# Pixie8888/R3DFSSeg

Measured on NVIDIA B200. Metric: MPTI episodes/s (2-way 5-shot, 2048 pts), higher is better.
Workload: dtype f32

## Files before the change

r3dfsseg_b200/csrc/api.cu:

```cuda
#include <stdlib.h>

#include "common.cuh"
#include "lp.cuh"
#include "proto.cuh"
#include "episode.cuh"

__global__ void gather_clouds_kernel(const float* __restrict__ x, int clouds_in, int C, int N,
                                     int64_t s_g, int64_t s_cloud, int64_t s_c, int64_t s_n,
                                     int cpe_out, int cloud_off, float* __restrict__ out,
                                     int64_t total) {
  const int64_t e = (int64_t)blockIdx.x * blockDim.x + threadIdx.x;
  if (e >= total) return;
  const int c = (int)(e % C);
  int64_t r = e / C;
  const int n = (int)(r % N);
  r /= N;
  const int cl = (int)(r % clouds_in);
  const int64_t grp = r / clouds_in;
  const int64_t ocloud = grp * cpe_out + cloud_off + cl;
  out[(ocloud * N + n) * C + c] = x[grp * s_g + cl * s_cloud + c * s_c + n * s_n];
}

__global__ void copy_cols_kernel(const float* __restrict__ src, int lds, int64_t M, int ncols,
                                 float* __restrict__ dst, int ldd, RowMap map) {
// ... 31 lines not shown
__global__ void proto_rows_kernel(const float* __restrict__ proto, int64_t p_e,
                                  const int32_t* __restrict__ proto_count, int64_t c_e, int S,
                                  int slot, int ppad, int64_t f_rows, float* __restrict__ F,
                                  int32_t* __restrict__ proto_cnt) {
  constexpr int D4 = R3DFS_FEAT_DIM / 4;
  const int e = blockIdx.y;
  const int i = blockIdx.x * blockDim.x + threadIdx.x;
  if (i < S) proto_cnt[e * S + i] = min(max(proto_count[e * c_e + i], 0), slot);
  if (i >= ppad * D4) return;
  const int r = i / D4, s = r / slot;
  int cnt = 0;
  if (s < S) cnt = min(max(proto_count[e * c_e + s], 0), slot);
  float4 v = make_float4(0.f, 0.f, 0.f, 0.f);
  if (r - s * slot < cnt) v = reinterpret_cast<const float4*>(proto + e * p_e)[i];
  reinterpret_cast<float4*>(F + e * f_rows * R3DFS_FEAT_DIM)[i] = v;
}

__global__ void i32_to_i64_kernel(const int32_t* __restrict__ a, int64_t* __restrict__ b,
                                  int64_t n) {
  const int64_t e = (int64_t)blockIdx.x * blockDim.x + threadIdx.x;
  if (e < n) b[e] = a[e];
}

thread_local long long r3dfs_launches = 0;

bool simt_gemm_forced() {
  static const bool v = [] {
    const char* e = R3DFS_GETENV("R3DFS_SIMT_GEMM");
    return e && e[0] == '1';
  }();
  return v;
}

int launch_knn_auto(const float* x, int ld, int C, const float* xx, int64_t B, int N, int k,
                    int32_t* idx32, int64_t* idx64, int impl, cudaStream_t st, void* split_ws,
                    size_t split_bytes) {
  if (impl == 2)
    return launch_knn_tc(x, ld, C, xx, B, N, k, idx32, idx64, st, split_ws, split_bytes);
  if (impl == 0 && !simt_gemm_forced() && C <= 64)
    return launch_knn_tc(x, ld, C, xx, B, N, k, idx32, idx64, st, split_ws, split_bytes);
  return launch_knn(x, ld, C, xx, B, N, k, idx32, idx64, st);
}

int launch_edge_mlp_auto(const float* PQ, const int32_t* idx, const float* w2, const float* s2,
                         const float* t2, int64_t B, int N, int k, float* Y, int ldy, RowMap map,
                         cudaStream_t st) {
  if (simt_gemm_forced())
    return launch_edge_mlp(PQ, idx, w2, s2, t2, B, N, k, Y, ldy, map, nullptr, st);
  return launch_edge_mlp_tc(PQ, idx, w2, s2, t2, B, N, k, Y, ldy, map, st);
}

int launch_attention_auto(const float* qkv, int ld, int64_t B, int N, float* Y, int ldy,
                          RowMap map, cudaStream_t st, float* kmax_ws, void* split_ws,
                          size_t split_bytes) {
  if (simt_gemm_forced()) return launch_attention(qkv, ld, B, N, Y, ldy, map, st);
  return launch_attention_tc(qkv, ld, B, N, Y, ldy, map, st, kmax_ws, split_ws, split_bytes);
}

int launch_linear_auto(const float* X, int ldx, const float* W, const float* s, const float* t,
                       int act, int64_t M, int K, int Nout, float* Y, int ldy, RowMap map,
                       cudaStream_t st) {
  if (simt_gemm_forced())
    return launch_linear(X, ldx, W, s, t, act, M, K, Nout, Y, ldy, map, st);
  const int rc = launch_linear_tma(X, ldx, W, s, t, act, M, K, Nout, Y, ldy, map, st);
  if (rc != R3DFS_E_UNSUPPORTED) return rc;
  return launch_linear_tc(X, ldx, W, s, t, act, M, K, Nout, Y, ldy, map, st);
}

static inline unsigned nblk(int64_t n, int t = 256) { return (unsigned)((n + t - 1) / t); }

void carve_encoder(WsBump& ws, int64_t M, int k, EncoderWs& e) {
  e.xx = ws.take<float>(M);
  e.idx = ws.take<int32_t>(M * k);
// ... 2 lines not shown
  e.tpq = ws.take<float>(128);
  e.PQ = ws.take<float>(M * 128);
  e.ecat = ws.take<float>(M * 192);
  e.h512 = ws.take<float>(M * 512);
  e.l2 = ws.take<float>(M * 256);
  e.h128 = ws.take<float>(M * 128);
  e.qkv = ws.take<float>(M * 192);
}

int check_weights(const r3dfs_weights_t* w) {
  if (!w) return R3DFS_E_BADARG;
  if (w->in_dim < 1 || w->in_dim > 64 || w->dgcnn_k < 1 || w->dgcnn_k > 32)
    return R3DFS_E_UNSUPPORTED;
  for (int i = 0; i < 3; ++i)
    if (!w->ec_w1[i] || !w->ec_s1[i] || !w->ec_t1[i] || !w->ec_w2[i] || !w->ec_s2[i] ||
        !w->ec_t2[i])
      return R3DFS_E_BADARG;
  for (int i = 0; i < 2; ++i)
    if (!w->mlp_w[i] || !w->mlp_s[i] || !w->mlp_t[i] || !w->bl_w[i] || !w->bl_s[i] || !w->bl_t[i])
      return R3DFS_E_BADARG;
  if (!w->att_wqkv) return R3DFS_E_BADARG;
  return 0;
}

int encoder_forward(const r3dfs_weights_t* w, const float* xp, int64_t B, int N,
                           const EncoderWs& e, float* F, RowMap map, float* level2,
                           cudaStream_t st, const StageRec* sr) {
  const int64_t M = B * N;
  const int k = w->dgcnn_k;
  for (int i = 0; i < 3; ++i) {
    const float* in = i == 0 ? xp : e.ecat + 64 * (i - 1);
    const int ld = i == 0 ? w->in_dim : 192;
    const int C = i == 0 ? w->in_dim : 64;
    R3DFS_TRY(launch_row_norms(in, M, ld, C, e.xx, st));
    R3DFS_TRY(launch_knn_auto(in, ld, C, e.xx, B, N, k, e.idx, nullptr, 0, st, e.h512,
                              sizeof(float) * (size_t)M * 512));
    if (sr) sr->mark(R3DFS_ST_KNN0 + 3 * i, st);
    R3DFS_TRY(launch_fold_edge_w1(w->ec_w1[i], w->ec_s1[i], w->ec_t1[i], C, e.wpq, e.spq, e.tpq, st));
    R3DFS_TRY(launch_linear_auto(in, ld, e.wpq, e.spq, e.tpq, ACT_NONE, M, C, 128, e.PQ, 128,
                            identity_map(), st));
    if (sr) sr->mark(R3DFS_ST_PQ0 + 3 * i, st);
    R3DFS_TRY(launch_edge_mlp_auto(e.PQ, e.idx, w->ec_w2[i], w->ec_s2[i], w->ec_t2[i], B, N, k,
                                   e.ecat + 64 * i, 192, identity_map(), st));
    if (sr) sr->mark(R3DFS_ST_EDGE0 + 3 * i, st);
  }
  copy_cols_kernel<<<nblk(M * 16), 256, 0, st>>>(e.ecat, 192, M, 64, F, 192, map);
  R3DFS_CHECK_LAUNCH();
  R3DFS_TRY(launch_linear_auto(e.ecat, 192, w->mlp_w[0], w->mlp_s[0], w->mlp_t[0], ACT_LRELU, M, 192,
                          512, e.h512, 512, identity_map(), st));
  R3DFS_TRY(launch_linear_auto(e.h512, 512, w->mlp_w[1], w->mlp_s[1], w->mlp_t[1], ACT_LRELU, M, 512,
                          256, e.l2, 256, identity_map(), st));
  if (sr) sr->mark(R3DFS_ST_MLP, st);
  if (level2) {
    cudaError_t ce = cudaMemcpyAsync(level2, e.l2, sizeof(float) * M * 256,
                                     cudaMemcpyDeviceToDevice, st);
    if (ce != cudaSuccess) return (int)ce;
  }
  R3DFS_TRY(launch_linear_auto(e.l2, 256, w->bl_w[0], w->bl_s[0], w->bl_t[0], ACT_RELU, M, 256, 128,
                          e.h128, 128, identity_map(), st));
  R3DFS_TRY(launch_linear_auto(e.h128, 128, w->bl_w[1], w->bl_s[1], w->bl_t[1], ACT_NONE, M, 128, 64,
                          F + 128, 192, map, st));
  if (sr) sr->mark(R3DFS_ST_BASE, st);
  R3DFS_TRY(launch_linear_auto(e.l2, 256, w->att_wqkv, nullptr, nullptr, ACT_NONE, M, 256, 192, e.qkv,
                          192, identity_map(), st));
  if (sr) sr->mark(R3DFS_ST_QKV, st);
  R3DFS_TRY(launch_attention_auto(e.qkv, 192, B, N, F + 64, 192, map, st, e.xx, e.h512,
                                  sizeof(float) * (size_t)M * 512));
// ... 14 lines not shown
    case R3DFS_E_UNSUPPORTED: return "shape not supported by the sm_100a kernels";
    case R3DFS_E_WORKSPACE: return "workspace too small";
    case R3DFS_E_ALIGN: return "pointer not 16-byte aligned";
    default: break;
  }
  if (code > 0) return cudaGetErrorString((cudaError_t)code);
  return "unknown error";
}

size_t r3dfs_knn_workspace(int64_t B, int64_t C, int64_t N, int k) {
  return align_up(sizeof(float) * B * N * C, 256) + align_up(sizeof(float) * B * N, 256) +
         align_up(knn_split_bytes((int)C, B, (int)N, k), 256) + 768;
}

int r3dfs_knn(const float* x, int64_t B, int64_t C, int64_t N, int64_t sb, int64_t sc, int64_t sn,
              int k, int64_t* idx_out, void* wsp, size_t ws_bytes, r3dfs_stream_t stream) {
  return r3dfs_knn_ex(x, B, C, N, sb, sc, sn, k, idx_out, 0, wsp, ws_bytes, stream);
}

int r3dfs_knn_ex(const float* x, int64_t B, int64_t C, int64_t N, int64_t sb, int64_t sc,
                 int64_t sn, int k, int64_t* idx_out, int impl, void* wsp, size_t ws_bytes,
                 r3dfs_stream_t stream) {
  if (!x || !idx_out || !wsp || B <= 0 || C <= 0 || N <= 0) return R3DFS_E_BADARG;
  if (k < 1 || k > 32 || k > N) return R3DFS_E_UNSUPPORTED;
  if (ws_bytes < r3dfs_knn_workspace(B, C, N, k)) return R3DFS_E_WORKSPACE;
  cudaStream_t st = (cudaStream_t)stream;
  WsBump ws(wsp, ws_bytes);
  float* xp = ws.take<float>(B * N * C);
  float* xx = ws.take<float>(B * N);
  const size_t split_bytes = knn_split_bytes((int)C, B, (int)N, k);
  unsigned char* split = split_bytes ? ws.take<unsigned char>(split_bytes) : nullptr;
  if (!ws.ok()) return R3DFS_E_WORKSPACE;
  R3DFS_TRY(launch_to_point_major(x, B, C, N, sb, sc, sn, xp, st));
  R3DFS_TRY(launch_row_norms(xp, B * N, (int)C, (int)C, xx, st));
  if (impl < 0 || impl > 2) return R3DFS_E_UNSUPPORTED;
  return launch_knn_auto(xp, (int)C, (int)C, xx, B, (int)N, k, nullptr, idx_out, impl, st, split,
                         split_bytes);
}

size_t r3dfs_edge_feature_workspace(int64_t B, int64_t C, int64_t N) {
  return edge_feature_scratch_bytes(B, C, N);
}

int r3dfs_edge_feature(const float* x, int64_t B, int64_t C, int64_t N, int64_t sb, int64_t sc,
                       int64_t sn, const int64_t* idx, int K, float* out, void* ws, size_t ws_bytes,
                       r3dfs_stream_t stream) {
  if (!x || !idx || !out || B <= 0 || C <= 0 || N <= 0 || K <= 0) return R3DFS_E_BADARG;
  if (C > 65535 || B > 65535) return R3DFS_E_UNSUPPORTED;
  if (((uintptr_t)out & 15) != 0) return R3DFS_E_ALIGN;
  return launch_edge_feature(x, B, C, N, sb, sc, sn, idx, K, out, (cudaStream_t)stream, ws, ws_bytes);
}

int r3dfs_linear_ex(const float* x, int64_t ldx, const float* w, const float* s, const float* t,
                    int act, int64_t M, int64_t K, int64_t Nout, float* y, int64_t ldy, int impl,
                    r3dfs_stream_t stream) {
  if (!x || !w || !y || M <= 0 || K <= 0 || Nout <= 0 || ldx < K || ldy < Nout)
    return R3DFS_E_BADARG;
  if (act < 0 || act > 2 || Nout > 65535 * 64 || impl < 0 || impl > 3) return R3DFS_E_UNSUPPORTED;
  cudaStream_t st = (cudaStream_t)stream;
  if (impl == 1)
    return launch_linear(x, (int)ldx, w, s, t, act, M, (int)K, (int)Nout, y, (int)ldy,
                         identity_map(), st);
  if (impl == 2)
    return launch_linear_tc(x, (int)ldx, w, s, t, act, M, (int)K, (int)Nout, y, (int)ldy,
                            identity_map(), st);
  if (impl == 3)
    return launch_linear_tma(x, (int)ldx, w, s, t, act, M, (int)K, (int)Nout, y, (int)ldy,
// ... 9 lines not shown
}

size_t r3dfs_edgeconv_workspace(int64_t B, int64_t C, int64_t N, int k) {
  const int64_t M = B * N;
  return align_up(sizeof(float) * M * C, 256) + align_up(sizeof(float) * M, 256) +
         align_up(sizeof(int32_t) * M * k, 256) + align_up(sizeof(float) * 128 * C, 256) +
         2 * 512 + align_up(sizeof(float) * M * 128, 256) +
         align_up(knn_split_bytes((int)C, B, (int)N, k), 256) + 1280;
}

int r3dfs_edgeconv(const float* x, int64_t B, int64_t C, int64_t N, int64_t sb, int64_t sc,
                   int64_t sn, int k, const float* w1, const float* s1, const float* t1,
                   const float* w2, const float* s2, const float* t2, float* y, int64_t* idx_out,
                   void* wsp, size_t ws_bytes, r3dfs_stream_t stream) {
  if (!x || !w1 || !s1 || !t1 || !w2 || !s2 || !t2 || !y || !wsp || B <= 0 || C <= 0 || N <= 0)
    return R3DFS_E_BADARG;
  if (k < 1 || k > 32 || k > N || B > 65535) return R3DFS_E_UNSUPPORTED;
  if (ws_bytes < r3dfs_edgeconv_workspace(B, C, N, k)) return R3DFS_E_WORKSPACE;
  if (((uintptr_t)y & 15) != 0) return R3DFS_E_ALIGN;
  cudaStream_t st = (cudaStream_t)stream;
  const int64_t M = B * N;
  WsBump ws(wsp, ws_bytes);
  float* xp = ws.take<float>(M * C);
  float* xx = ws.take<float>(M);
  int32_t* idx = ws.take<int32_t>(M * k);
  float* wpq = ws.take<float>(128 * C);
  float* spq = ws.take<float>(128);
  float* tpq = ws.take<float>(128);
  float* PQ = ws.take<float>(M * 128);
  const size_t split_bytes = knn_split_bytes((int)C, B, (int)N, k);
  unsigned char* split = split_bytes ? ws.take<unsigned char>(split_bytes) : nullptr;
  if (!ws.ok()) return R3DFS_E_WORKSPACE;
  R3DFS_TRY(launch_to_point_major(x, B, C, N, sb, sc, sn, xp, st));
  R3DFS_TRY(launch_row_norms(xp, M, (int)C, (int)C, xx, st));
  R3DFS_TRY(launch_knn_auto(xp, (int)C, (int)C, xx, B, (int)N, k, idx, idx_out, 0, st, split,
                            split_bytes));
  R3DFS_TRY(launch_fold_edge_w1(w1, s1, t1, (int)C, wpq, spq, tpq, st));
  R3DFS_TRY(launch_linear_auto(xp, (int)C, wpq, spq, tpq, ACT_NONE, M, (int)C, 128, PQ, 128,
                               identity_map(), st));
  return launch_edge_mlp_auto(PQ, idx, w2, s2, t2, B, (int)N, k, y, 64, identity_map(), st);
}

size_t r3dfs_attention_workspace(int64_t B, int64_t N) {
  return align_up(sizeof(float) * B * N * 192, 256) + align_up(sizeof(float) * B, 256) +
         align_up(attention_split_bytes(B, (int)N), 256) + 512;
}

int r3dfs_attention(const float* x, int64_t B, int64_t N, int64_t Cin, const float* wqkv, float* y,
                    void* wsp, size_t ws_bytes, r3dfs_stream_t stream) {
  if (!x || !wqkv || !y || !wsp || B <= 0 || N <= 0 || Cin <= 0) return R3DFS_E_BADARG;
  if (B > 65535) return R3DFS_E_UNSUPPORTED;
  if (ws_bytes < r3dfs_attention_workspace(B, N)) return R3DFS_E_WORKSPACE;
  cudaStream_t st = (cudaStream_t)stream;
  WsBump ws(wsp, ws_bytes);
  float* qkv = ws.take<float>(B * N * 192);
  float* kmax = ws.take<float>(B);
  const size_t split_bytes = attention_split_bytes(B, (int)N);
  unsigned char* split = ws.take<unsigned char>(split_bytes);
  if (!ws.ok()) return R3DFS_E_WORKSPACE;
  R3DFS_TRY(launch_linear_auto(x, (int)Cin, wqkv, nullptr, nullptr, ACT_NONE, B * N, (int)Cin, 192,
                               qkv, 192, identity_map(), st));
  return launch_attention_auto(qkv, 192, B, (int)N, y, 64, identity_map(), st, kmax, split,
                               split_bytes);
}

size_t r3dfs_features_workspace(int64_t B, int64_t N) {
  const int64_t M = B * N;
// ... 654 lines not shown
```

r3dfsseg_b200/csrc/common.cuh:

```cuda
#pragma once
#include <cuda_runtime.h>
#include <stdint.h>
#include <math.h>

#include "../../include/r3dfs.h"

#define R3DFS_FEAT_DIM 192
#define R3DFS_EC_WIDTH 64

extern thread_local long long r3dfs_launches;

#ifdef R3DFS_AB_SWITCHES
#include <stdlib.h>
#define R3DFS_GETENV(name) getenv(name)
#else
#define R3DFS_GETENV(name) ((const char*)nullptr)
#endif

#define R3DFS_CHECK_LAUNCH()                       \
  do {                                             \
    cudaError_t e__ = cudaGetLastError();          \
    if (e__ != cudaSuccess) return (int)e__;       \
    ++r3dfs_launches;                              \
  } while (0)
// ... 41 lines not shown
  int cpe;
  int n;
  int64_t ep_rows;
  int64_t row_off;
  __host__ __device__ inline int64_t operator()(int64_t m) const {
    if (cpe == 0) return m;
    int64_t b = m / n, i = m - b * n;
    return (b / cpe) * ep_rows + row_off + (b % cpe) * (int64_t)n + i;
  }
};
static inline RowMap identity_map() { return RowMap{0, 1, 0, 0}; }

enum Act { ACT_NONE = 0, ACT_RELU = 1, ACT_LRELU = 2 };

__device__ __forceinline__ float apply_act(float v, int act) {
  if (act == ACT_RELU) return fmaxf(v, 0.f);
  if (act == ACT_LRELU) return v > 0.f ? v : 0.2f * v;
  return v;
}

__device__ __forceinline__ float warp_sum(float v) {
#pragma unroll
  for (int o = 16; o > 0; o >>= 1) v += __shfl_xor_sync(0xffffffffu, v, o);
  return v;
}

int launch_to_point_major(const float* x, int64_t B, int64_t C, int64_t N, int64_t sb, int64_t sc,
                          int64_t sn, float* out, cudaStream_t st);
int launch_row_norms(const float* x, int64_t rows, int ld, int C, float* out, cudaStream_t st);
int launch_row_norms_batched(const float* x, int64_t xs, int batch, int64_t rows, int ld, int C,
                             float* out, cudaStream_t st);
int launch_knn(const float* x, int ld, int C, const float* xx, int64_t B, int N, int k,
               int32_t* idx32, int64_t* idx64, cudaStream_t st);
int launch_knn_tc(const float* x, int ld, int C, const float* xx, int64_t B, int N, int k,
                  int32_t* idx32, int64_t* idx64, cudaStream_t st, void* split_ws = nullptr,
                  size_t split_bytes = 0);
size_t knn_split_bytes(int C, int64_t B, int N, int k);
int launch_knn_auto(const float* x, int ld, int C, const float* xx, int64_t B, int N, int k,
                    int32_t* idx32, int64_t* idx64, int impl, cudaStream_t st,
                    void* split_ws = nullptr, size_t split_bytes = 0);
int launch_linear(const float* X, int ldx, const float* W, const float* s, const float* t, int act,
                  int64_t M, int K, int Nout, float* Y, int ldy, RowMap map, cudaStream_t st);
int launch_linear_tc(const float* X, int ldx, const float* W, const float* s, const float* t,
                     int act, int64_t M, int K, int Nout, float* Y, int ldy, RowMap map,
                     cudaStream_t st);
int launch_linear_tma(const float* X, int ldx, const float* W, const float* s, const float* t,
                      int act, int64_t M, int K, int Nout, float* Y, int ldy, RowMap map,
                      cudaStream_t st);
int launch_linear_auto(const float* X, int ldx, const float* W, const float* s, const float* t,
                       int act, int64_t M, int K, int Nout, float* Y, int ldy, RowMap map,
                       cudaStream_t st);
int launch_gram_dist_ts(const float* F, int64_t graph_rows, int64_t row_off, int G, int nn, int D,
                        const float* norms, float* D2, cudaStream_t st);
int launch_gram_dist_tc(const float* F, int64_t graph_rows, int64_t row_off, int G, int nn, int D,
                        const float* norms, float* D2, cudaStream_t st);
int launch_edge_mlp_tc(const float* PQ, const int32_t* idx, const float* w2, const float* s2,
                       const float* t2, int64_t B, int N, int k, float* Y, int ldy, RowMap map,
                       cudaStream_t st);
int launch_edge_mlp_auto(const float* PQ, const int32_t* idx, const float* w2, const float* s2,
                         const float* t2, int64_t B, int N, int k, float* Y, int ldy, RowMap map,
                         cudaStream_t st);
bool simt_gemm_forced();
int launch_edge_mlp(const float* PQ, const int32_t* idx, const float* w2, const float* s2,
                    const float* t2, int64_t B, int N, int k, float* Y, int ldy, RowMap map,
                    float* w2t_scratch, cudaStream_t st);
int launch_edge_feature(const float* x, int64_t B, int64_t C, int64_t N, int64_t sb, int64_t sc,
                        int64_t sn, const int64_t* idx, int K, float* out, cudaStream_t st,
                        void* ws = nullptr, size_t ws_bytes = 0);
size_t edge_feature_scratch_bytes(int64_t B, int64_t C, int64_t N);
int launch_attention(const float* qkv, int ld, int64_t B, int N, float* Y, int ldy, RowMap map,
                     cudaStream_t st);
// ... 18 lines not shown
```

r3dfsseg_b200/csrc/tc_knn.cu:

```cuda
#include <stdlib.h>

#include "common.cuh"
#include "tc.cuh"

#define KT_TQ 128
#define KT_TC 128
#define KT_THREADS 384

template <int KC4>
struct KnnTcSmem {
  static constexpr int TILE = tc::tile_bytes(128, KC4);
  static constexpr int Q_OFF = 0;
  static constexpr int B_OFF = 2 * TILE;
  static constexpr int QV_OFF = B_OFF + 4 * TILE;
  static constexpr int QI_OFF = QV_OFF + 16 * 256 * 4;
  static constexpr int XS_OFF = QI_OFF + 16 * 256;
  static constexpr int TOTAL = XS_OFF + 4 * 128 * 4 + 64;
};

template <int KC4>
__device__ __forceinline__ void knn_store_tile(unsigned char* hi_base, unsigned char* lo_base,
                                               const float* __restrict__ x, int ld, int C,
                                               int64_t row0, int64_t rows_end, int t, int nthr,
                                               bool vec_ok) {
// ... 57 lines not shown
template <int KC4, int ROWS, int NTHR>
__device__ __forceinline__ void tile_store(const TileRegs<KC4, ROWS, NTHR>& tr,
                                           unsigned char* hi_base, unsigned char* lo_base, int t) {
  constexpr int LBO = tc::tile_lbo(ROWS);
#pragma unroll
  for (int i = 0; i < TileRegs<KC4, ROWS, NTHR>::NCH; ++i) {
    const int c = t + i * NTHR;
    const int r = c / KC4, kc = c % KC4;
    float4 hi, lo;
    tc::split4(tr.v[i], hi, lo);
    *reinterpret_cast<float4*>(hi_base + kc * LBO + r * 16) = hi;
    *reinterpret_cast<float4*>(lo_base + kc * LBO + r * 16) = lo;
  }
}

__device__ __forceinline__ void mbar_arrive(uint64_t* bar) {
  asm volatile("mbarrier.arrive.shared::cta.b64 _, [%0];" ::"r"(tc::smem_u32(bar)) : "memory");
}

template <int KL>
__device__ __forceinline__ void list_insert(float (&lv)[KL], int (&li)[KL], float key, int idx) {
#pragma unroll
  for (int i = KL - 1; i > 0; --i) {
    const bool up = key > lv[i - 1];
    const bool here = key > lv[i];
    const float nv = up ? lv[i - 1] : (here ? key : lv[i]);
    const int ni = up ? li[i - 1] : (here ? idx : li[i]);
    lv[i] = nv;
    li[i] = ni;
  }
  if (key > lv[0]) {
    lv[0] = key;
    li[0] = idx;
  }
}

template <int KC4, int KL>
__global__ __launch_bounds__(KT_THREADS, 1) void knn_tc_kernel(const float* __restrict__ x, int ld,
                                                               int C, const float* __restrict__ xx,
                                                               int N, int k,
                                                               int32_t* __restrict__ idx32,
                                                               int64_t* __restrict__ idx64) {
  extern __shared__ __align__(128) unsigned char smem[];
  using S = KnnTcSmem<KC4>;
  __shared__ uint64_t bar_full[2];
  __shared__ uint64_t bar_tfree[2];
  __shared__ uint32_t tmem_base_s;
  const int tid = threadIdx.x, lane = tid & 31, w = tid >> 5;
  const int b = blockIdx.y;
  const int q0 = blockIdx.x * KT_TQ;
  const int64_t base = (int64_t)b * N;
  constexpr int LBO = tc::tile_lbo(128);
  constexpr uint32_t IDESC = tc::make_idesc_tf32(128, KT_TC);
  const bool vec_ok = ((ld & 3) == 0) && ((reinterpret_cast<uintptr_t>(x) & 15) == 0);
  const int T = (N + KT_TC - 1) / KT_TC;
  const int ksteps = (min(C, 4 * KC4) + 7) / 8;

  if (tid == 0) {
    tc::mbar_init(&bar_full[0], 1);
    tc::mbar_init(&bar_full[1], 1);
    tc::mbar_init(&bar_tfree[0], 256);
    tc::mbar_init(&bar_tfree[1], 256);
    tc::mbar_fence_init();
  }
  if (w == 0) tc::tmem_alloc(&tmem_base_s, 2 * KT_TC);
  knn_store_tile<KC4>(smem + S::Q_OFF, smem + S::Q_OFF + S::TILE, x, ld, C, base + q0, base + N,
// ... 470 lines not shown
static int launch_knn_tc2_t(const float* x, int ld, int C, const float* xx, int64_t B, int N, int k,
                            int32_t* idx32, int64_t* idx64, cudaStream_t st) {
  using S = Knn2Smem<KC4>;
  cudaError_t e = cudaFuncSetAttribute(knn_tc2_kernel<KC4>,
                                       cudaFuncAttributeMaxDynamicSharedMemorySize, S::TOTAL);
  if (e != cudaSuccess) return (int)e;
  dim3 grid((N + KT_TQ - 1) / KT_TQ, (unsigned)B);
  knn_tc2_kernel<KC4><<<grid, K2_THREADS, S::TOTAL, st>>>(x, ld, C, xx, N, k, idx32, idx64);
  R3DFS_CHECK_LAUNCH();
  return 0;
}

#ifdef KNN_TRACE
__device__ long long g_knn_trace[8 * 4096];
#define KNN_TR(slot, j) \
  do { if (blockIdx.x == KNN_TRACE_BX && blockIdx.y == KNN_TRACE_BY) g_knn_trace[(slot) * 4096 + (j)] = clock64(); } while (0)
#else
#define KNN_TR(slot, j) do { } while (0)
#endif
#define K3_THREADS 576
#define K3_TC 128
#define K3_NACC 3
#define K3_NR 8
#define K3_APPROX1(kc4) ((kc4) >= 16)
#define K3_G 16

template <int KC4>
struct KnnSplit {
  static constexpr int TB = tc::tile_bytes(K3_TC, KC4);
  static constexpr int NORMS = K3_TC * 4 + 16;
  static constexpr int BLK = 2 * TB + NORMS;
};

template <int KC4>
__global__ __launch_bounds__(256) void knn_split_kernel(const float* __restrict__ x, int ld, int C,
                                                        const float* __restrict__ xx, int N,
                                                        unsigned char* __restrict__ out) {
  extern __shared__ __align__(128) unsigned char sm[];
  using P = KnnSplit<KC4>;
  constexpr int LBO = tc::tile_lbo(K3_TC);
  const int t = blockIdx.x, b = blockIdx.y, tid = threadIdx.x;
  const int T = gridDim.x;
  const int64_t base = (int64_t)b * N;
  const bool vec_ok = ((ld & 3) == 0) && ((reinterpret_cast<uintptr_t>(x) & 15) == 0);
  knn_store_tile_r<KC4, K3_TC>(sm, sm + P::TB, x, ld, C, base + (int64_t)t * K3_TC, base + N, tid,
                               256, vec_ok);
  if (tid < K3_TC) {
    const int cn = t * K3_TC + tid;
    const float nv = cn < N ? xx[base + cn] : 0.f;
    float* nrm = reinterpret_cast<float*>(sm + 2 * P::TB);
    nrm[tid] = nv;
    float mx = nv;
#pragma unroll
    for (int o = 16; o > 0; o >>= 1) mx = fmaxf(mx, __shfl_xor_sync(0xffffffffu, mx, o));
    if ((tid & 31) == 0) nrm[K3_TC + (tid >> 5)] = mx;
  }
  if (tid < 2 * KC4)
    *reinterpret_cast<float4*>(sm + (tid / KC4) * P::TB + (tid % KC4) * LBO + K3_TC * 16) =
        make_float4(0.f, 0.f, 0.f, 0.f);
  __syncthreads();
  float4* dst = reinterpret_cast<float4*>(out + ((int64_t)b * T + t) * P::BLK);
  const float4* src = reinterpret_cast<const float4*>(sm);
  for (int i = tid; i < P::BLK / 16; i += 256) dst[i] = src[i];
}

template <int KC4, int NST, int CAP>
struct Knn3Smem {
  static constexpr int TB = tc::tile_bytes(K3_TC, KC4);
  static constexpr int B_OFF = 0;
  static constexpr int XS_OFF = B_OFF + NST * 2 * TB;
  static constexpr int QK_OFF = XS_OFF + K3_NR * (K3_TC * 4 + 16);
  static constexpr int QC_OFF = QK_OFF + CAP * 512 * 4;
  static constexpr int TOTAL = QC_OFF + CAP * 512 * 2;
  static_assert(CAP >= K3_G + 1 && CAP >= 17, "queue region: pass-1 group maxima / half a chunk");
  static_assert(NST * 2 * TB >= 3 * 20 * 128 * 8, "the final merge borrows the operand stages");
};

__device__ __forceinline__ void sort16_desc(float (&v)[16]) {
#pragma unroll
  for (int size = 2; size <= 16; size <<= 1) {
#pragma unroll
    for (int stride = size >> 1; stride > 0; stride >>= 1) {
#pragma unroll
      for (int i = 0; i < 16; ++i) {
        const int j = i ^ stride;
        if (j > i) {
          const bool desc = (i & size) == 0;
          const float a = v[i], b = v[j];
          v[i] = desc ? fmaxf(a, b) : fminf(a, b);
          v[j] = desc ? fminf(a, b) : fmaxf(a, b);
        }
      }
    }
  }
}

template <int KC4, int NST, int CAP>
__global__ __launch_bounds__(K3_THREADS, 1) void knn_tc3_kernel(
    const float* __restrict__ x, int ld, int C, const float* __restrict__ xx,
    const unsigned char* __restrict__ split, int N, int k, int32_t* __restrict__ idx32,
    int64_t* __restrict__ idx64) {
  constexpr int KL = 20;
  constexpr int QCOLS = 8 * KC4;
  constexpr int ACC0 = 128;
  extern __shared__ __align__(128) unsigned char smem[];
  using S = Knn3Smem<KC4, NST, CAP>;
  using P = KnnSplit<KC4>;
  static_assert(QCOLS <= ACC0, "query operand overlaps the accumulators");
  __shared__ uint64_t bar_sfull[NST];
  __shared__ uint64_t bar_sfree[NST];
  __shared__ uint64_t bar_full[K3_NACC];
  __shared__ uint64_t bar_tfree[K3_NACC];
  __shared__ uint64_t bar_q[2];
  __shared__ uint32_t tmem_base_s;
  const int tid = threadIdx.x, lane = tid & 31, w = tid >> 5;
  const int b = blockIdx.y;
  const int q0 = blockIdx.x * KT_TQ;
  const int64_t base = (int64_t)b * N;
  constexpr int LBOB = tc::tile_lbo(K3_TC);
  constexpr uint32_t IDESC = tc::make_idesc_tf32(128, K3_TC);
  const int T = (N + K3_TC - 1) / K3_TC;
  const int ksteps = (min(C, 4 * KC4) + 7) / 8;
  if (tid == 0) KNN_TR(6, 4000);

  if (tid == 0) {
    for (int i = 0; i < NST; ++i) {
      tc::mbar_init(&bar_sfull[i], 1);
      tc::mbar_init(&bar_sfree[i], 1);
    }
    for (int i = 0; i < K3_NACC; ++i) {
// ... 68 lines not shown
      if (j >= K3_NACC) tc::mbar_wait(&bar_tfree[a], ((j / K3_NACC) - 1) & 1);
      if (lane == 0) KNN_TR(2, j);
      tc::tc_fence_after();
      const uint32_t b_hi = tc::smem_u32(smem + S::B_OFF + s * 2 * S::TB), b_lo = b_hi + S::TB;
      const uint32_t d = tmem_d + ACC0 + a * K3_TC;
      const uint64_t dbh = tc::make_desc(b_hi, LBOB, 128), dbl = tc::make_desc(b_lo, LBOB, 128);
      if (K3_APPROX1(KC4) && j < T) {
        tc::mma_tf32_ts_elect<false>(d, aq_hi, dbh, IDESC);
#pragma unroll
        for (int ks = 1; ks < 2 * KC4 / 4; ++ks)
          if (ks < ksteps) tc::mma_tf32_ts_elect<true>(d, aq_hi + 8 * ks, dbh + ks * KB, IDESC);
      } else {
        tc::mma_tf32_ts_elect<false>(d, aq_lo, dbh, IDESC);
        tc::mma_tf32_ts_elect<true>(d, aq_hi, dbl, IDESC);
        tc::mma_tf32_ts_elect<true>(d, aq_hi, dbh, IDESC);
#pragma unroll
        for (int ks = 1; ks < 2 * KC4 / 4; ++ks) {
          if (ks < ksteps) {
            tc::mma_tf32_ts_elect<true>(d, aq_lo + 8 * ks, dbh + ks * KB, IDESC);
            tc::mma_tf32_ts_elect<true>(d, aq_hi + 8 * ks, dbl + ks * KB, IDESC);
            tc::mma_tf32_ts_elect<true>(d, aq_hi + 8 * ks, dbh + ks * KB, IDESC);
          }
        }
      }
      tc::mma_commit_elect(&bar_sfree[s]);
      tc::mma_commit_elect(&bar_full[a]);
      if (lane == 0) KNN_TR(3, j);
    }
  } else {
    float* qk = reinterpret_cast<float*>(smem + S::QK_OFF);
    unsigned short* qc = reinterpret_cast<unsigned short*>(smem + S::QC_OFF);
    const int row = 32 * (w & 3) + lane;
    const int cq = w >> 2;
    const int q = q0 + row;
    const float nq = (q < N) ? -xx[base + q] : 0.f;
    const unsigned char* xs_ring = smem + S::XS_OFF;
    const uint32_t taddr = tmem_d + ((uint32_t)(32 * (w & 3)) << 16) + (uint32_t)(ACC0 + 32 * cq);
    float kmax2 = 0.f;
#pragma unroll 1
    for (int s = 0; s < K3_G; ++s) qk[s * 512 + tid] = -INFINITY;
#pragma unroll 1
    for (int j = 0; j < T; ++j) {
      const int a = j % K3_NACC;
      if (tid == 0) KNN_TR(7, j);
      tc::mbar_wait(&bar_full[a], (j / K3_NACC) & 1);
      if (tid == 0) KNN_TR(4, j);
      tc::tc_fence_after();
      float v[32];
      tc::tmem_ld32(taddr + (uint32_t)(a * K3_TC), v);
      if (tid == 0) KNN_TR(5, j);
      const int c0 = j * K3_TC + 32 * cq;
      {
        const float* xs = reinterpret_cast<const float*>(xs_ring + (j & (K3_NR - 1)) * P::NORMS);
        knn_keys32(v, nq, xs + 32 * cq);
        if (K3_APPROX1(KC4)) {
          const float4 tm = *reinterpret_cast<const float4*>(xs + K3_TC);
          kmax2 = fmaxf(kmax2, fmaxf(fmaxf(tm.x, tm.y), fmaxf(tm.z, tm.w)));
        }
      }
      tc::tc_fence_before();
      mbar_arrive(&bar_tfree[a]);
      if (tid == 0) KNN_TR(6, j);
      float m = -INFINITY;
      if (c0 + 32 <= N) {
#pragma unroll
        for (int e = 0; e < 32; ++e) m = fmaxf(m, v[e]);
      } else {
#pragma unroll
// ... 68 lines not shown
      mbar_arrive(&bar_tfree[a]);
      if (tid == 0) KNN_TR(6, j);
      const int nvalid = N - c0;
#pragma unroll
      for (int hh = 0; hh < 32; hh += 16) {
        if (__any_sync(0xffffffffu, qcnt > CAP - 16)) drain();
        const float thr = lv[KL - 1];
        const int tb = __float_as_int(thr);
        const float cut = fmaxf(tau, __int_as_float(tb >= 0 ? tb + 1 : (tb == (int)0x80000000 ? 1 : tb - 1)));
        if (nvalid >= 32) {
#pragma unroll
          for (int e = hh; e < hh + 16; ++e) {
            if (v[e] >= cut) {
              qk[qcnt * 512 + tid] = v[e];
              qc[qcnt * 512 + tid] = (unsigned short)(c0 + e);
              ++qcnt;
            }
          }
        } else {
#pragma unroll
          for (int e = hh; e < hh + 16; ++e) {
            if (v[e] >= cut && e < nvalid) {
              qk[qcnt * 512 + tid] = v[e];
              qc[qcnt * 512 + tid] = (unsigned short)(c0 + e);
              ++qcnt;
            }
          }
        }
      }
    }
    if (tid == 0) KNN_TR(6, 4002);
    drain();
    if (tid == 0) KNN_TR(6, 4003);
    float* mv = reinterpret_cast<float*>(smem + S::B_OFF);
    int* mi = reinterpret_cast<int*>(smem + S::B_OFF) + 3 * KL * 128;
    asm volatile("bar.sync 2, 512;" ::: "memory");
    if (cq & 1) {
#pragma unroll
      for (int i = 0; i < KL; ++i) {
        mv[((cq >> 1) * KL + i) * 128 + row] = lv[i];
        mi[((cq >> 1) * KL + i) * 128 + row] = li[i];
      }
    }
    asm volatile("bar.sync 2, 512;" ::: "memory");
    if (!(cq & 1)) {
#pragma unroll 1
      for (int i = 0; i < KL; ++i) {
        const float key = mv[((cq >> 1) * KL + i) * 128 + row];
        if (!(key > lv[KL - 1])) break;
        list_insert<KL>(lv, li, key, mi[((cq >> 1) * KL + i) * 128 + row]);
      }
      if (cq == 2) {
#pragma unroll
        for (int i = 0; i < KL; ++i) {
          mv[(2 * KL + i) * 128 + row] = lv[i];
          mi[(2 * KL + i) * 128 + row] = li[i];
        }
      }
    }
    asm volatile("bar.sync 2, 512;" ::: "memory");
    if (cq == 0) {
#pragma unroll 1
      for (int i = 0; i < KL; ++i) {
        const float key = mv[(2 * KL + i) * 128 + row];
        if (!(key > lv[KL - 1])) break;
        list_insert<KL>(lv, li, key, mi[(2 * KL + i) * 128 + row]);
      }
      if (q < N) {
#pragma unroll
        for (int i = 0; i < KL; ++i) {
          if (i < k) {
            const int64_t o = (base + q) * k + i;
            if (idx32) idx32[o] = li[i];
            if (idx64) idx64[o] = li[i];
          }
        }
      }
    }
  }
  if (tid == 0) KNN_TR(6, 4004);
  tc::tc_fence_before();
  __syncthreads();
  if (w == 0) tc::tmem_dealloc(tmem_d, 512);
  if (tid == 0) KNN_TR(6, 4005);
}

template <int KC4, int NST, int CAP>
static int launch_knn_tc3_t(const float* x, int ld, int C, const float* xx, int64_t B, int N, int k,
                            int32_t* idx32, int64_t* idx64, void* split_ws, cudaStream_t st) {
  using S = Knn3Smem<KC4, NST, CAP>;
  using P = KnnSplit<KC4>;
  static_assert(S::TOTAL <= 232448 - 256, "shared memory budget");
  const int T = (N + K3_TC - 1) / K3_TC;
  cudaError_t e = cudaFuncSetAttribute(knn_split_kernel<KC4>,
                                       cudaFuncAttributeMaxDynamicSharedMemorySize, P::BLK);
  if (e != cudaSuccess) return (int)e;
  knn_split_kernel<KC4><<<dim3(T, (unsigned)B), 256, P::BLK, st>>>(x, ld, C, xx, N,
                                                                   (unsigned char*)split_ws);
  R3DFS_CHECK_LAUNCH();
  e = cudaFuncSetAttribute(knn_tc3_kernel<KC4, NST, CAP>,
                           cudaFuncAttributeMaxDynamicSharedMemorySize, S::TOTAL);
  if (e != cudaSuccess) return (int)e;
  dim3 grid((N + KT_TQ - 1) / KT_TQ, (unsigned)B);
  knn_tc3_kernel<KC4, NST, CAP><<<grid, K3_THREADS, S::TOTAL, st>>>(
      x, ld, C, xx, (const unsigned char*)split_ws, N, k, idx32, idx64);
  R3DFS_CHECK_LAUNCH();
  return 0;
}

size_t knn_split_bytes(int C, int64_t B, int N, int k) {
  if (k < 1 || k > 20 || C > 64 || N < 1024 || N > 65535 || N < k) return 0;
  const size_t T = (size_t)(N + K3_TC - 1) / K3_TC;
  const size_t blk = C <= 16 ? KnnSplit<4>::BLK : KnnSplit<16>::BLK;
  return (size_t)B * T * blk;
}

template <int KC4, int KL>
static int launch_knn_tc_t(const float* x, int ld, int C, const float* xx, int64_t B, int N, int k,
                           int32_t* idx32, int64_t* idx64, cudaStream_t st) {
  using S = KnnTcSmem<KC4>;
  cudaError_t e = cudaFuncSetAttribute(knn_tc_kernel<KC4, KL>,
                                       cudaFuncAttributeMaxDynamicSharedMemorySize, S::TOTAL);
  if (e != cudaSuccess) return (int)e;
  dim3 grid((N + KT_TQ - 1) / KT_TQ, (unsigned)B);
  knn_tc_kernel<KC4, KL><<<grid, KT_THREADS, S::TOTAL, st>>>(x, ld, C, xx, N, k, idx32, idx64);
  R3DFS_CHECK_LAUNCH();
  return 0;
}

static bool knn_single_pass_forced() {
  static const bool v = [] {
    const char* e = R3DFS_GETENV("R3DFS_KNN_SINGLE_PASS");
    return e && e[0] == '1';
  }();
  return v;
}

static bool knn_tc2_forced() {
  static const bool v = [] {
    const char* e = R3DFS_GETENV("R3DFS_KNN_TC2");
    return e && e[0] == '1';
  }();
  return v;
}

int launch_knn_tc(const float* x, int ld, int C, const float* xx, int64_t B, int N, int k,
                  int32_t* idx32, int64_t* idx64, cudaStream_t st, void* split_ws,
                  size_t split_bytes) {
  if (k < 1 || k > 32 || C > 64 || N < k) return R3DFS_E_UNSUPPORTED;
  if (split_ws && !knn_single_pass_forced() && !knn_tc2_forced()) {
    const size_t need = knn_split_bytes(C, B, N, k);
    if (need && split_bytes >= need && (reinterpret_cast<uintptr_t>(split_ws) & 15) == 0) {
      if (C <= 16)
        return launch_knn_tc3_t<4, 4, 30>(x, ld, C, xx, B, N, k, idx32, idx64, split_ws, st);
      return launch_knn_tc3_t<16, 2, 30>(x, ld, C, xx, B, N, k, idx32, idx64, split_ws, st);
    }
  }
  if (k <= 20 && N >= 1024 && N <= 65535 && !knn_single_pass_forced()) {
    if (C <= 16) return launch_knn_tc2_t<4>(x, ld, C, xx, B, N, k, idx32, idx64, st);
    return launch_knn_tc2_t<16>(x, ld, C, xx, B, N, k, idx32, idx64, st);
  }
  if (C <= 16) {
    if (k <= 20) return launch_knn_tc_t<4, 20>(x, ld, C, xx, B, N, k, idx32, idx64, st);
    return launch_knn_tc_t<4, 32>(x, ld, C, xx, B, N, k, idx32, idx64, st);
  }
  if (k <= 20) return launch_knn_tc_t<16, 20>(x, ld, C, xx, B, N, k, idx32, idx64, st);
  return launch_knn_tc_t<16, 32>(x, ld, C, xx, B, N, k, idx32, idx64, st);
}
```

r3dfsseg_b200/csrc/train_api.cu:

```cuda
#include "episode.cuh"
#include "lp.cuh"
#include "proto.cuh"
#include "train.cuh"

#define BN_EPS 1e-5f
#define BN_MOMENTUM 0.1f
#define CONTRAST_FPS_K 4
#define CONTRAST_TEMP 0.1f
#define SGEMM_PARTIAL_FLOATS ((size_t)8 << 20)
#define BN_SCRATCH_DOUBLES ((size_t)2 * 512 * BN_MAX_BLOCKS + 2 * 512)

static const int kBnChannels[R3DFS_N_BN] = {64, 64, 64, 64, 64, 64, 512, 256, 128, 64};

static void param_layout(int in_dim, int64_t* off) {
  int64_t o = 0;
  int i = 0;
  for (int l = 0; l < 3; ++l) {
    const int C = l == 0 ? in_dim : 64;
    const int64_t sz[6] = {64 * 2 * (int64_t)C, 64, 64, 64 * 64, 64, 64};
    for (int q = 0; q < 6; ++q) {
      off[i++] = o;
      o += sz[q];
    }
  }
// ... 202 lines not shown
  bi = gi + 1;
  return 0;
}

static int bn_fwd(const TrainCtx& c, const TrainWs& t, const GroupWs& g, int b, const float* x,
                  int64_t ldx, int64_t rows, int act, float* y, int64_t ldy) {
  int gi, bi;
  bn_index_param(b, gi, bi);
  const int C = kBnChannels[b];
  R3DFS_TRY(launch_bn_stats(x, ldx, rows, C, BN_EPS, BN_MOMENTUM, c.R(b), g.stats[b], t.bn_scratch,
                            c.st));
  return launch_bn_act(x, ldx, rows, C, g.stats[b], c.P(gi), c.P(bi), act, y, ldy, c.st);
}

static int bn_bwd(const TrainCtx& c, const TrainWs& t, const GroupWs& g, int b, const float* dy,
                  int64_t ld_dy, const float* x, int64_t ldx, int64_t rows, int act, float* dx,
                  int64_t ld_dx) {
  int gi, bi;
  bn_index_param(b, gi, bi);
  return launch_bn_act_bwd(dy, ld_dy, x, ldx, rows, kBnChannels[b], g.stats[b], c.P(gi), c.P(bi), act,
                           dx, ld_dx, c.G(gi), c.G(bi), t.bn_scratch, c.st);
}

static int group_forward(const TrainCtx& c, const TrainWs& t, const GroupWs& g, float dropout_p,
                         const uint8_t* keep, float* Fout) {
  const int N = c.N, k = c.k;
  const int64_t M = g.M, Ek = g.Ek;
  cudaStream_t st = c.st;
  for (int i = 0; i < 3; ++i) {
    const float* in = i == 0 ? g.xp : g.ecat + 64 * (i - 1);
    const int ld = i == 0 ? c.in_dim : 192;
    const int C = i == 0 ? c.in_dim : 64;
    const int pw = 6 * i;
    R3DFS_TRY(launch_row_norms(in, M, ld, C, t.xx, st));
    R3DFS_TRY(launch_knn_auto(in, ld, C, t.xx, g.B, N, k, g.idx[i], nullptr, 0, st));
    R3DFS_TRY(lin_fwd(c, in, ld, t.wpq[i], nullptr, M, C, 128, t.PQ, 128));
    R3DFS_TRY(launch_edge_pre(t.PQ, g.idx[i], g.B, N, k, g.h1pre[i], st));
    R3DFS_TRY(bn_fwd(c, t, g, 2 * i, g.h1pre[i], 64, Ek, ACT_LRELU, t.edgeA, 64));
    R3DFS_TRY(lin_fwd(c, t.edgeA, 64, c.P(pw + R3DFS_P_EC0_W2), nullptr, Ek, 64, 64, g.h2pre[i], 64));
    int gi, bi;
    bn_index_param(2 * i + 1, gi, bi);
    R3DFS_TRY(launch_bn_stats(g.h2pre[i], 64, Ek, 64, BN_EPS, BN_MOMENTUM, c.R(2 * i + 1),
                              g.stats[2 * i + 1], t.bn_scratch, st));
    R3DFS_TRY(launch_edge_max(g.h2pre[i], g.stats[2 * i + 1], c.P(gi), c.P(bi), M, k,
                              g.ecat + 64 * i, 192, g.arg[i], st));
  }
  R3DFS_TRY(launch_copy_cols_plain(g.ecat, 192, M, 64, Fout, 192, st));
  R3DFS_TRY(lin_fwd(c, g.ecat, 192, c.P(R3DFS_P_MLP0_W), nullptr, M, 192, 512, g.h512pre, 512));
  R3DFS_TRY(bn_fwd(c, t, g, 6, g.h512pre, 512, M, ACT_LRELU, g.a512, 512));
  R3DFS_TRY(lin_fwd(c, g.a512, 512, c.P(R3DFS_P_MLP1_W), nullptr, M, 512, 256, g.l2pre, 256));
  R3DFS_TRY(bn_fwd(c, t, g, 7, g.l2pre, 256, M, ACT_LRELU, g.l2, 256));
  R3DFS_TRY(lin_fwd(c, g.l2, 256, c.P(R3DFS_P_BL0_W), c.P(R3DFS_P_BL0_BIAS), M, 256, 128, g.bl0pre, 128));
  R3DFS_TRY(bn_fwd(c, t, g, 8, g.bl0pre, 128, M, ACT_RELU, g.bl0a, 128));
  R3DFS_TRY(lin_fwd(c, g.bl0a, 128, c.P(R3DFS_P_BL1_W), c.P(R3DFS_P_BL1_BIAS), M, 128, 64, g.bl1pre, 64));
  R3DFS_TRY(bn_fwd(c, t, g, 9, g.bl1pre, 64, M, ACT_NONE, Fout + 128, 192));
  R3DFS_TRY(lin_fwd(c, g.l2, 256, c.P(R3DFS_P_ATT_Q), nullptr, M, 256, 192, g.qkv, 192));
  const int64_t cs = (int64_t)N * 192, ps = (int64_t)N * N;
  R3DFS_TRY(launch_sgemm(g.qkv, 192, 1, cs, g.qkv + 64, 1, 192, cs, g.P, N, ps, N, N, 64, (int)g.B,
                         0.125f, 0.f, 1, t.partial, st));
  const bool drop = keep != nullptr && dropout_p > 0.f;
  R3DFS_TRY(launch_softmax_rows(g.P, g.B * N, N, drop ? keep : nullptr, dropout_p, g.Pd, st));
  const float* Pd = drop ? g.Pd : g.P;
  R3DFS_TRY(launch_sgemm(Pd, N, 1, ps, g.qkv + 128, 192, 1, cs, Fout + 64, 192, cs, N, 64, N,
                         (int)g.B, 1.f, 0.f, 1, t.partial, st));
  return 0;
}

// ... 362 lines not shown
```

Measured before the change: 945.1.

## Fuse row norms into kNN split kernel and use merge-path final list merge

Row norms are now computed inside the kNN split kernel from the tile already staged in shared memory, and the main tc3 kernel reads them from the split buffer. This removes the separate row-norm launch and its global read of the points in every kNN call. The final cross-warp top-k merge is replaced by a two-level merge of sorted lists that goes through shared memory borrowed from the queue region, in place of repeated early-exit insertions. The old path is kept behind an environment flag, and row-norm launches move inside the fallback paths.

```diff
diff --git a/r3dfsseg_b200/csrc/api.cu b/r3dfsseg_b200/csrc/api.cu
--- a/r3dfsseg_b200/csrc/api.cu
+++ b/r3dfsseg_b200/csrc/api.cu
@@ -87,13 +87,14 @@
   return v;
 }
 
-int launch_knn_auto(const float* x, int ld, int C, const float* xx, int64_t B, int N, int k,
+int launch_knn_auto(const float* x, int ld, int C, float* xx, int64_t B, int N, int k,
                     int32_t* idx32, int64_t* idx64, int impl, cudaStream_t st, void* split_ws,
                     size_t split_bytes) {
   if (impl == 2)
     return launch_knn_tc(x, ld, C, xx, B, N, k, idx32, idx64, st, split_ws, split_bytes);
   if (impl == 0 && !simt_gemm_forced() && C <= 64)
     return launch_knn_tc(x, ld, C, xx, B, N, k, idx32, idx64, st, split_ws, split_bytes);
+  R3DFS_TRY(launch_row_norms(x, B * N, ld, C, xx, st));
   return launch_knn(x, ld, C, xx, B, N, k, idx32, idx64, st);
 }
 
@@ -162,7 +163,6 @@
     const float* in = i == 0 ? xp : e.ecat + 64 * (i - 1);
     const int ld = i == 0 ? w->in_dim : 192;
     const int C = i == 0 ? w->in_dim : 64;
-    R3DFS_TRY(launch_row_norms(in, M, ld, C, e.xx, st));
     R3DFS_TRY(launch_knn_auto(in, ld, C, e.xx, B, N, k, e.idx, nullptr, 0, st, e.h512,
                               sizeof(float) * (size_t)M * 512));
     if (sr) sr->mark(R3DFS_ST_KNN0 + 3 * i, st);
@@ -243,7 +243,6 @@
   unsigned char* split = split_bytes ? ws.take<unsigned char>(split_bytes) : nullptr;
   if (!ws.ok()) return R3DFS_E_WORKSPACE;
   R3DFS_TRY(launch_to_point_major(x, B, C, N, sb, sc, sn, xp, st));
-  R3DFS_TRY(launch_row_norms(xp, B * N, (int)C, (int)C, xx, st));
   if (impl < 0 || impl > 2) return R3DFS_E_UNSUPPORTED;
   return launch_knn_auto(xp, (int)C, (int)C, xx, B, (int)N, k, nullptr, idx_out, impl, st, split,
                          split_bytes);
@@ -319,7 +318,6 @@
   unsigned char* split = split_bytes ? ws.take<unsigned char>(split_bytes) : nullptr;
   if (!ws.ok()) return R3DFS_E_WORKSPACE;
   R3DFS_TRY(launch_to_point_major(x, B, C, N, sb, sc, sn, xp, st));
-  R3DFS_TRY(launch_row_norms(xp, M, (int)C, (int)C, xx, st));
   R3DFS_TRY(launch_knn_auto(xp, (int)C, (int)C, xx, B, (int)N, k, idx, idx_out, 0, st, split,
                             split_bytes));
   R3DFS_TRY(launch_fold_edge_w1(w1, s1, t1, (int)C, wpq, spq, tpq, st));
diff --git a/r3dfsseg_b200/csrc/common.cuh b/r3dfsseg_b200/csrc/common.cuh
--- a/r3dfsseg_b200/csrc/common.cuh
+++ b/r3dfsseg_b200/csrc/common.cuh
@@ -97,11 +97,11 @@
                              float* out, cudaStream_t st);
 int launch_knn(const float* x, int ld, int C, const float* xx, int64_t B, int N, int k,
                int32_t* idx32, int64_t* idx64, cudaStream_t st);
-int launch_knn_tc(const float* x, int ld, int C, const float* xx, int64_t B, int N, int k,
+int launch_knn_tc(const float* x, int ld, int C, float* xx, int64_t B, int N, int k,
                   int32_t* idx32, int64_t* idx64, cudaStream_t st, void* split_ws = nullptr,
                   size_t split_bytes = 0);
 size_t knn_split_bytes(int C, int64_t B, int N, int k);
-int launch_knn_auto(const float* x, int ld, int C, const float* xx, int64_t B, int N, int k,
+int launch_knn_auto(const float* x, int ld, int C, float* xx, int64_t B, int N, int k,
                     int32_t* idx32, int64_t* idx64, int impl, cudaStream_t st,
                     void* split_ws = nullptr, size_t split_bytes = 0);
 int launch_linear(const float* X, int ldx, const float* W, const float* s, const float* t, int act,
diff --git a/r3dfsseg_b200/csrc/tc_knn.cu b/r3dfsseg_b200/csrc/tc_knn.cu
--- a/r3dfsseg_b200/csrc/tc_knn.cu
+++ b/r3dfsseg_b200/csrc/tc_knn.cu
@@ -113,6 +113,21 @@
   if (key > lv[0]) {
     lv[0] = key;
     li[0] = idx;
+  }
+}
+
+template <int KL>
+__device__ __forceinline__ void merge_lists(const float* av, const int* ai, const float* bv,
+                                            const int* bi, float (&lv)[KL], int (&li)[KL]) {
+  int ia = 0, ib = 0;
+#pragma unroll
+  for (int i = 0; i < KL; ++i) {
+    const float a = av[ia * 128], b = bv[ib * 128];
+    const bool tb = b > a;
+    lv[i] = tb ? b : a;
+    li[i] = tb ? bi[ib * 128] : ai[ia * 128];
+    ia += tb ? 0 : 1;
+    ib += tb ? 1 : 0;
   }
 }
 
@@ -649,7 +664,7 @@
   static constexpr int BLK = 2 * TB + NORMS;
 };
 
-template <int KC4>
+template <int KC4, bool V1>
 __global__ __launch_bounds__(256) void knn_split_kernel(const float* __restrict__ x, int ld, int C,
                                                         const float* __restrict__ xx, int N,
                                                         unsigned char* __restrict__ out) {
@@ -662,11 +677,40 @@
   const bool vec_ok = ((ld & 3) == 0) && ((reinterpret_cast<uintptr_t>(x) & 15) == 0);
   knn_store_tile_r<KC4, K3_TC>(sm, sm + P::TB, x, ld, C, base + (int64_t)t * K3_TC, base + N, tid,
                                256, vec_ok);
+  float* nrm = reinterpret_cast<float*>(sm + 2 * P::TB);
+  if (!V1) {
+    __syncthreads();
+    if (tid < K3_TC) {
+      float p[32];
+#pragma unroll
+      for (int l = 0; l < 32; ++l) p[l] = 0.f;
+#pragma unroll
+      for (int kc = 0; kc < KC4; ++kc) {
+        const float4 h = *reinterpret_cast<const float4*>(sm + kc * LBO + tid * 16);
+        const float4 l = *reinterpret_cast<const float4*>(sm + P::TB + kc * LBO + tid * 16);
+        const float v[4] = {h.x + l.x, h.y + l.y, h.z + l.z, h.w + l.w};
+#pragma unroll
+        for (int e = 0; e < 4; ++e) {
+          const int c = 4 * kc + e;
+          p[c & 31] = fmaf(v[e], v[e], p[c & 31]);
+        }
+      }
+#pragma unroll
+      for (int o = 16; o > 0; o >>= 1)
+#pragma unroll
+        for (int l = 0; l < o; ++l) p[l] = p[l] + p[l + o];
+      nrm[tid] = p[0];
+    }
+  }
   if (tid < K3_TC) {
     const int cn = t * K3_TC + tid;
-    const float nv = cn < N ? xx[base + cn] : 0.f;
-    float* nrm = reinterpret_cast<float*>(sm + 2 * P::TB);
-    nrm[tid] = nv;
+    float nv;
+    if (!V1) {
+      nv = nrm[tid];
+    } else {
+      nv = cn < N ? xx[base + cn] : 0.f;
+      nrm[tid] = nv;
+    }
     float mx = nv;
 #pragma unroll
     for (int o = 16; o > 0; o >>= 1) mx = fmaxf(mx, __shfl_xor_sync(0xffffffffu, mx, o));
@@ -690,7 +734,8 @@
   static constexpr int QC_OFF = QK_OFF + CAP * 512 * 4;
   static constexpr int TOTAL = QC_OFF + CAP * 512 * 2;
   static_assert(CAP >= K3_G + 1 && CAP >= 17, "queue region: pass-1 group maxima / half a chunk");
-  static_assert(NST * 2 * TB >= 3 * 20 * 128 * 8, "the final merge borrows the operand stages");
+  static_assert(NST * 2 * TB >= 3 * 20 * 128 * 8 && NST * 2 * TB >= 4 * 20 * 128 * 4 &&
+                CAP * 512 * 4 >= 4 * 20 * 128 * 4, "the final merge borrows the operand stages and queue");
 };
 
 __device__ __forceinline__ void sort16_desc(float (&v)[16]) {
@@ -712,7 +757,7 @@
   }
 }
 
-template <int KC4, int NST, int CAP>
+template <int KC4, int NST, int CAP, bool V1>
 __global__ __launch_bounds__(K3_THREADS, 1) void knn_tc3_kernel(
     const float* __restrict__ x, int ld, int C, const float* __restrict__ xx,
     const unsigned char* __restrict__ split, int N, int k, int32_t* __restrict__ idx32,
@@ -847,8 +892,12 @@
     unsigned short* qc = reinterpret_cast<unsigned short*>(smem + S::QC_OFF);
     const int row = 32 * (w & 3) + lane;
     const int cq = w >> 2;
-    const int q = q0 + row;
-    const float nq = (q < N) ? -xx[base + q] : 0.f;
+    const bool q_ok = row < N - q0;
+    float nq = 0.f;
+    if (q_ok)
+      nq = V1 ? -xx[base + q0 + row]
+              : -reinterpret_cast<const float*>(split + ((int64_t)b * T + blockIdx.x) * P::BLK +
+                                                2 * S::TB)[row];
     const unsigned char* xs_ring = smem + S::XS_OFF;
     const uint32_t taddr = tmem_d + ((uint32_t)(32 * (w & 3)) << 16) + (uint32_t)(ACC0 + 32 * cq);
     float kmax2 = 0.f;
@@ -983,45 +1032,71 @@
     if (tid == 0) KNN_TR(6, 4002);
     drain();
     if (tid == 0) KNN_TR(6, 4003);
-    float* mv = reinterpret_cast<float*>(smem + S::B_OFF);
-    int* mi = reinterpret_cast<int*>(smem + S::B_OFF) + 3 * KL * 128;
-    asm volatile("bar.sync 2, 512;" ::: "memory");
-    if (cq & 1) {
+    if (!V1) {
+      float* mv = reinterpret_cast<float*>(smem + S::B_OFF);
+      int* mi = reinterpret_cast<int*>(smem + S::QK_OFF);
+      float* pv = mv + cq * KL * 128 + row;
+      int* pi = mi + cq * KL * 128 + row;
+      asm volatile("bar.sync 2, 512;" ::: "memory");
 #pragma unroll
       for (int i = 0; i < KL; ++i) {
-        mv[((cq >> 1) * KL + i) * 128 + row] = lv[i];
-        mi[((cq >> 1) * KL + i) * 128 + row] = li[i];
-      }
-    }
-    asm volatile("bar.sync 2, 512;" ::: "memory");
-    if (!(cq & 1)) {
+        pv[i * 128] = lv[i];
+        pi[i * 128] = li[i];
+      }
+      asm volatile("bar.sync 2, 512;" ::: "memory");
+      if (!(cq & 1)) {
+        merge_lists<KL>(pv, pi, pv + KL * 128, pi + KL * 128, lv, li);
+#pragma unroll
+        for (int i = 0; i < KL; ++i) {
+          pv[i * 128] = lv[i];
+          pi[i * 128] = li[i];
+        }
+      }
+      asm volatile("bar.sync 2, 512;" ::: "memory");
+      if (cq == 0) merge_lists<KL>(pv, pi, pv + 2 * KL * 128, pi + 2 * KL * 128, lv, li);
+    } else {
+      float* mv = reinterpret_cast<float*>(smem + S::B_OFF);
+      int* mi = reinterpret_cast<int*>(smem + S::B_OFF) + 3 * KL * 128;
+      asm volatile("bar.sync 2, 512;" ::: "memory");
+      if (cq & 1) {
+#pragma unroll
+        for (int i = 0; i < KL; ++i) {
+          mv[((cq >> 1) * KL + i) * 128 + row] = lv[i];
+          mi[((cq >> 1) * KL + i) * 128 + row] = li[i];
+        }
+      }
+      asm volatile("bar.sync 2, 512;" ::: "memory");
+      if (!(cq & 1)) {
 #pragma unroll 1
-      for (int i = 0; i < KL; ++i) {
-        const float key = mv[((cq >> 1) * KL + i) * 128 + row];
-        if (!(key > lv[KL - 1])) break;
-        list_insert<KL>(lv, li, key, mi[((cq >> 1) * KL + i) * 128 + row]);
-      }
-      if (cq == 2) {
-#pragma unroll
         for (int i = 0; i < KL; ++i) {
-          mv[(2 * KL + i) * 128 + row] = lv[i];
-          mi[(2 * KL + i) * 128 + row] = li[i];
-        }
-      }
-    }
-    asm volatile("bar.sync 2, 512;" ::: "memory");
+          const float key = mv[((cq >> 1) * KL + i) * 128 + row];
+          if (!(key > lv[KL - 1])) break;
+          list_insert<KL>(lv, li, key, mi[((cq >> 1) * KL + i) * 128 + row]);
+        }
+        if (cq == 2) {
+#pragma unroll
+          for (int i = 0; i < KL; ++i) {
+            mv[(2 * KL + i) * 128 + row] = lv[i];
+            mi[(2 * KL + i) * 128 + row] = li[i];
+          }
+        }
+      }
+      asm volatile("bar.sync 2, 512;" ::: "memory");
+      if (cq == 0) {
+#pragma unroll 1
+        for (int i = 0; i < KL; ++i) {
+          const float key = mv[(2 * KL + i) * 128 + row];
+          if (!(key > lv[KL - 1])) break;
+          list_insert<KL>(lv, li, key, mi[(2 * KL + i) * 128 + row]);
+        }
+      }
+    }
     if (cq == 0) {
-#pragma unroll 1
-      for (int i = 0; i < KL; ++i) {
-        const float key = mv[(2 * KL + i) * 128 + row];
-        if (!(key > lv[KL - 1])) break;
-        list_insert<KL>(lv, li, key, mi[(2 * KL + i) * 128 + row]);
-      }
-      if (q < N) {
+      if (q_ok) {
 #pragma unroll
         for (int i = 0; i < KL; ++i) {
           if (i < k) {
-            const int64_t o = (base + q) * k + i;
+            const int64_t o = (base + q0 + row) * k + i;
             if (idx32) idx32[o] = li[i];
             if (idx64) idx64[o] = li[i];
           }
@@ -1036,24 +1111,24 @@
   if (tid == 0) KNN_TR(6, 4005);
 }
 
-template <int KC4, int NST, int CAP>
+template <int KC4, int NST, int CAP, bool V1>
 static int launch_knn_tc3_t(const float* x, int ld, int C, const float* xx, int64_t B, int N, int k,
                             int32_t* idx32, int64_t* idx64, void* split_ws, cudaStream_t st) {
   using S = Knn3Smem<KC4, NST, CAP>;
   using P = KnnSplit<KC4>;
   static_assert(S::TOTAL <= 232448 - 256, "shared memory budget");
   const int T = (N + K3_TC - 1) / K3_TC;
-  cudaError_t e = cudaFuncSetAttribute(knn_split_kernel<KC4>,
+  cudaError_t e = cudaFuncSetAttribute(knn_split_kernel<KC4, V1>,
                                        cudaFuncAttributeMaxDynamicSharedMemorySize, P::BLK);
   if (e != cudaSuccess) return (int)e;
-  knn_split_kernel<KC4><<<dim3(T, (unsigned)B), 256, P::BLK, st>>>(x, ld, C, xx, N,
-                                                                   (unsigned char*)split_ws);
+  knn_split_kernel<KC4, V1><<<dim3(T, (unsigned)B), 256, P::BLK, st>>>(x, ld, C, xx, N,
+                                                                          (unsigned char*)split_ws);
   R3DFS_CHECK_LAUNCH();
-  e = cudaFuncSetAttribute(knn_tc3_kernel<KC4, NST, CAP>,
+  e = cudaFuncSetAttribute(knn_tc3_kernel<KC4, NST, CAP, V1>,
                            cudaFuncAttributeMaxDynamicSharedMemorySize, S::TOTAL);
   if (e != cudaSuccess) return (int)e;
   dim3 grid((N + KT_TQ - 1) / KT_TQ, (unsigned)B);
-  knn_tc3_kernel<KC4, NST, CAP><<<grid, K3_THREADS, S::TOTAL, st>>>(
+  knn_tc3_kernel<KC4, NST, CAP, V1><<<grid, K3_THREADS, S::TOTAL, st>>>(
       x, ld, C, xx, (const unsigned char*)split_ws, N, k, idx32, idx64);
   R3DFS_CHECK_LAUNCH();
   return 0;
@@ -1087,6 +1162,14 @@
   return v;
 }
 
+static bool knn_tc3_v1_forced() {
+  static const bool v = [] {
+    const char* e = R3DFS_GETENV("R3DFS_KNN_TC3_V1");
+    return e && e[0] == '1';
+  }();
+  return v;
+}
+
 static bool knn_tc2_forced() {
   static const bool v = [] {
     const char* e = R3DFS_GETENV("R3DFS_KNN_TC2");
@@ -1095,18 +1178,25 @@
   return v;
 }
 
-int launch_knn_tc(const float* x, int ld, int C, const float* xx, int64_t B, int N, int k,
+int launch_knn_tc(const float* x, int ld, int C, float* xx, int64_t B, int N, int k,
                   int32_t* idx32, int64_t* idx64, cudaStream_t st, void* split_ws,
                   size_t split_bytes) {
   if (k < 1 || k > 32 || C > 64 || N < k) return R3DFS_E_UNSUPPORTED;
   if (split_ws && !knn_single_pass_forced() && !knn_tc2_forced()) {
     const size_t need = knn_split_bytes(C, B, N, k);
     if (need && split_bytes >= need && (reinterpret_cast<uintptr_t>(split_ws) & 15) == 0) {
+      if (knn_tc3_v1_forced()) {
+        R3DFS_TRY(launch_row_norms(x, B * N, ld, C, xx, st));
+        if (C <= 16)
+          return launch_knn_tc3_t<4, 4, 30, true>(x, ld, C, xx, B, N, k, idx32, idx64, split_ws, st);
+        return launch_knn_tc3_t<16, 2, 30, true>(x, ld, C, xx, B, N, k, idx32, idx64, split_ws, st);
+      }
       if (C <= 16)
-        return launch_knn_tc3_t<4, 4, 30>(x, ld, C, xx, B, N, k, idx32, idx64, split_ws, st);
-      return launch_knn_tc3_t<16, 2, 30>(x, ld, C, xx, B, N, k, idx32, idx64, split_ws, st);
-    }
-  }
+        return launch_knn_tc3_t<4, 4, 30, false>(x, ld, C, xx, B, N, k, idx32, idx64, split_ws, st);
+      return launch_knn_tc3_t<16, 2, 30, false>(x, ld, C, xx, B, N, k, idx32, idx64, split_ws, st);
+    }
+  }
+  R3DFS_TRY(launch_row_norms(x, B * N, ld, C, xx, st));
   if (k <= 20 && N >= 1024 && N <= 65535 && !knn_single_pass_forced()) {
     if (C <= 16) return launch_knn_tc2_t<4>(x, ld, C, xx, B, N, k, idx32, idx64, st);
     return launch_knn_tc2_t<16>(x, ld, C, xx, B, N, k, idx32, idx64, st);
diff --git a/r3dfsseg_b200/csrc/train_api.cu b/r3dfsseg_b200/csrc/train_api.cu
--- a/r3dfsseg_b200/csrc/train_api.cu
+++ b/r3dfsseg_b200/csrc/train_api.cu
@@ -258,7 +258,6 @@
     const int ld = i == 0 ? c.in_dim : 192;
     const int C = i == 0 ? c.in_dim : 64;
     const int pw = 6 * i;
-    R3DFS_TRY(launch_row_norms(in, M, ld, C, t.xx, st));
     R3DFS_TRY(launch_knn_auto(in, ld, C, t.xx, g.B, N, k, g.idx[i], nullptr, 0, st));
     R3DFS_TRY(lin_fwd(c, in, ld, t.wpq[i], nullptr, M, C, 128, t.PQ, 128));
     R3DFS_TRY(launch_edge_pre(t.PQ, g.idx[i], g.B, N, k, g.h1pre[i], st));
```

After: 968.2, median of 6. +2.4%, better.
